# Walter0807/MotionBERT

Hardware: AMD Instinct MI355X
Metric: clips/sec [B,243,17,3] DSTformer fwd+bwd (higher is better)
Workload: dtype bf16; 1 GPU; MotionBERT full DSTformer (dim_feat 512, depth 5, 8 heads, mlp_ratio 2) train step: fwd + bwd + AdamW, 64 clips/GPU x T=243 x J=17, random-init weights, pose loss (mpjpe + 0.5 n_mpjpe + 20 velocity, fused kernel), one-launch flat AdamW; global_batch=64, frames=243, parallelism=dp1

## Files before the change

### motionbert_amd/csrc/attention.hip

```cpp
#include "attention_common.h"

template <bool SHARED> struct AttnBlock { static constexpr int THREADS = SHARED ? 512 : 256, WAVES = THREADS / 64; };
constexpr int MBX_ATTN_KV_THREADS = 256;
template <bool SHARED> struct AttnBlockKV { static constexpr int THREADS = SHARED ? MBX_ATTN_KV_THREADS : 256, WAVES = THREADS / 64; };


template <typename T, int HD, bool SHARED, bool DROP = false>
__global__ __launch_bounds__(AttnBlock<SHARED>::THREADS, (sizeof(T) == 2 && !DROP) ? 4 : 1) void attn_fwd_kernel(const T* __restrict__ qkv, T* __restrict__ o, float* __restrict__ lse,
                                                       int Tn, int J, int H, float scale, int mode, int nprob, int KP, MbxDrop dr) {
    constexpr bool IS_BF = sizeof(T) == 2;
    constexpr int KSTR = rm_stride<T>(HD);
    extern __shared__ __attribute__((aligned(16))) char smem[];
    const int tid = threadIdx.x, lane = tid & 63, wave = tid >> 6, g = lane >> 5;
    const int C = H * HD, C3 = 3 * C;
    constexpr int VSTR = KSTR;
    const int KBYTES = KP * KSTR;
    const int VBYTES = KP * VSTR;
    int prob = SHARED ? (int)blockIdx.x : (int)blockIdx.x * 4 + wave;
    const bool pvalid = prob < nprob;
    prob = min(prob, nprob - 1);
    const Prob P = decode_prob(prob, mode, Tn, J, H);
    const int gtid = SHARED ? tid : lane, gsize = SHARED ? AttnBlock<SHARED>::THREADS : 64;
    char* kt = smem + (SHARED ? 0 : wave * (KBYTES + VBYTES));
    char* vt = kt + KBYTES;
// ... 398 lines not shown
                a1 = wave_halves<WaveAdd>(a1); a2 = wave_halves<WaveAdd>(a2);
                b1 = wave_halves<WaveAdd>(b1); b2 = wave_halves<WaveAdd>(b2);
                if (rvalid && g == 0) {
                    const size_t Mtot = (size_t)(nprob / H) * P.L;
                    *reinterpret_cast<float2*>(st_part + ((size_t)(2 * P.h) * Mtot + tok) * 2) = make_float2(a1, a2);
                    *reinterpret_cast<float2*>(st_part + ((size_t)(2 * P.h + 1) * Mtot + tok) * 2) = make_float2(b1, b2);
                }
            }
        }
        if (!stats) {
            store_rowfrag<T, HD>(reinterpret_cast<T*>(vt + (size_t)i * RSTR), dk, 1.0f, g);
            store_rowfrag<T, HD>(reinterpret_cast<T*>(qt + (size_t)i * RSTR), dv, 1.0f, g);
        }
    }
    if (pvalid) {
        constexpr int CH = HD * (int)sizeof(T) / 16;
        T* ob = dqkv + P.tok0 * C3 + (size_t)P.h * HD;
        const char* sa = stats ? qt : kt;
        const char* sb = stats ? kt : vt;
        const char* sc = stats ? vt : qt;
        for (int idx = lane; idx < P.L * CH; idx += 64) {
            const int r = idx / CH, ch = idx % CH, off = r * RSTR + ch * 16;
            const uint4 a = *reinterpret_cast<const uint4*>(sa + off);
            const uint4 b = *reinterpret_cast<const uint4*>(sb + off);
            const uint4 c = *reinterpret_cast<const uint4*>(sc + off);
            if (sizeof(T) == 4 && dq_lo) {
                const size_t eo = P.tok0 * C3 + (size_t)P.h * HD + (size_t)r * rstride + ch * 4;
                bf16_t* const hi = reinterpret_cast<bf16_t*>(dqkv);
                const float va[4] = {__uint_as_float(a.x), __uint_as_float(a.y), __uint_as_float(a.z), __uint_as_float(a.w)};
                const float vb[4] = {__uint_as_float(b.x), __uint_as_float(b.y), __uint_as_float(b.z), __uint_as_float(b.w)};
                const float vc[4] = {__uint_as_float(c.x), __uint_as_float(c.y), __uint_as_float(c.z), __uint_as_float(c.w)};
                store4_planes(hi + eo, dq_lo + eo, va);
                store4_planes(hi + eo + C, dq_lo + eo + C, vb);
                store4_planes(hi + eo + 2 * C, dq_lo + eo + 2 * C, vc);
                continue;
            }
            T* dst = ob + (size_t)r * rstride + ch * (16 / (int)sizeof(T));
            *reinterpret_cast<uint4*>(dst) = a;
            *reinterpret_cast<uint4*>(dst + C) = b;
            *reinterpret_cast<uint4*>(dst + 2 * C) = c;
        }
    }
}

__device__ __forceinline__ bf16_t* qt_row(char* tile, int row, int stride) { return reinterpret_cast<bf16_t*>(tile + (size_t)row * stride); }
template <int HD>
__device__ __forceinline__ void mma_rows_ldsb(const char* tile, int stride, int row0, const char* brow, int lane, f32x16_t& acc) {
    const char* p = tile + (size_t)(row0 + (lane & 31)) * stride + (lane >> 5) * 16;
#pragma unroll
    for (int s = 0; s < HD / 16; ++s) {
        const bf16x8_t a = *reinterpret_cast<const bf16x8_t*>(p + s * 32);
        const bf16x8_t b = *reinterpret_cast<const bf16x8_t*>(brow + s * 32);
        acc = __builtin_amdgcn_mfma_f32_32x32x16_bf16(a, b, acc, 0, 0, 0);
    }
}

struct Raw4b {
    static __device__ __forceinline__ void unpack(const uint2& r, float (&v)[4]) {
        v[0] = __uint_as_float(r.x << 16); v[1] = __uint_as_float(r.x & 0xffff0000u);
        v[2] = __uint_as_float(r.y << 16); v[3] = __uint_as_float(r.y & 0xffff0000u);
    }
};
#ifndef MBX_ATTN_DBG
#define MBX_ATTN_DBG 0
#endif
#ifdef MBX_ATTN_TRACE
__device__ long long* g_attn_trace;
#define AT_TS(slot_) do { if (threadIdx.x == 0) ats[slot_] = (long long)wall_clock64(); __builtin_amdgcn_sched_barrier(0); } while (0)
#else
#define AT_TS(slot_) do { } while (0)
#endif
template <int HD, bool STATS>
__global__ __launch_bounds__(1024, 1) void attn_bwd_fused_kernel(const bf16_t* __restrict__ qkv, const bf16_t* __restrict__ o,
                                                                 const bf16_t* __restrict__ d_o, const float* __restrict__ lse,
                                                                 bf16_t* __restrict__ dqkv, int Tn, int J, int H, float scale,
                                                                 int mode, int nprob, int KP, const float* __restrict__ st_bias,
                                                                 const float* __restrict__ st_rsum, float* __restrict__ st_part) {
    typedef bf16_t T;
    constexpr int RSTR = rm_stride<T>(HD), CH = HD / 8;
    extern __shared__ __attribute__((aligned(16))) char smem[];
#ifdef MBX_ATTN_TRACE
    long long ats[8] = {0, 0, 0, 0, 0, 0, 0, 0};
#endif
    AT_TS(0);
    const int tid = threadIdx.x, lane = tid & 63, wave = __builtin_amdgcn_readfirstlane(tid >> 6), g = lane >> 5;
    const int C = H * HD, C3 = 3 * C;
    const Prob P = decode_prob((int)blockIdx.x, mode, Tn, J, H);
    const int TB = KP * RSTR;
    char* qt = smem;
    char* kt = qt + TB;
    char* vt = kt + TB;
    char* dot_ = vt + TB;
    float* lse_s = reinterpret_cast<float*>(dot_ + TB);
    float* del_s = lse_s + KP;
    uint4* vec = reinterpret_cast<uint4*>(del_s + KP);
    const size_t rstride = (size_t)P.tstep * C3, ostride = (size_t)P.tstep * C;
    const T* qbase = qkv + P.tok0 * C3 + (size_t)P.h * HD;
    const T* dobase = d_o + P.tok0 * C + (size_t)P.h * HD;
    const T* obase = o + P.tok0 * C + (size_t)P.h * HD;
    if (STATS) fill_stat_vec<HD>(vec, st_rsum, st_bias, C, P.h, tid, 1024);

    for (int i0 = tid; i0 < KP * CH; i0 += 2048) {
        uint4 v[2][4], vo[2];
        float sl[2] = {0.f, 0.f};
#pragma unroll
        for (int u = 0; u < 2; ++u) {
            const int idx = i0 + u * 1024, row = idx / CH, ch = idx % CH;
#pragma unroll
            for (int t = 0; t < 4; ++t) v[u][t] = make_uint4(0u, 0u, 0u, 0u);
            vo[u] = make_uint4(0u, 0u, 0u, 0u);
            if (idx < KP * CH && row < P.L && !(MBX_ATTN_DBG & 4)) {
                const T* r3 = qbase + (size_t)row * rstride + ch * 8;
                v[u][0] = *reinterpret_cast<const uint4*>(r3);
                v[u][1] = *reinterpret_cast<const uint4*>(r3 + C);
                v[u][2] = *reinterpret_cast<const uint4*>(r3 + 2 * C);
                v[u][3] = *reinterpret_cast<const uint4*>(dobase + (size_t)row * ostride + ch * 8);
                vo[u] = *reinterpret_cast<const uint4*>(obase + (size_t)row * ostride + ch * 8);
                if (ch == 0) sl[u] = lse[(P.tok0 + (size_t)row * P.tstep) * H + P.h];
            }
        }
#pragma unroll
        for (int u = 0; u < 2; ++u) {
            const int idx = i0 + u * 1024, row = idx / CH, ch = idx % CH;
            if (idx < KP * CH) {
                const int off = row * RSTR + ch * 16;
                *reinterpret_cast<uint4*>(qt + off) = v[u][0];
                *reinterpret_cast<uint4*>(kt + off) = v[u][1];
                *reinterpret_cast<uint4*>(vt + off) = v[u][2];
                *reinterpret_cast<uint4*>(dot_ + off) = v[u][3];
            }
        }
        AT_TS(1);
#pragma unroll
        for (int u = 0; u < 2; ++u) {
            const int idx = i0 + u * 1024, row = idx / CH, ch = idx % CH;
            float x[4], y[4], dl = 0.f;
            Raw4b::unpack(make_uint2(v[u][3].x, v[u][3].y), x); Raw4b::unpack(make_uint2(vo[u].x, vo[u].y), y);
            dl = fmaf(x[0], y[0], fmaf(x[1], y[1], fmaf(x[2], y[2], fmaf(x[3], y[3], dl))));
            Raw4b::unpack(make_uint2(v[u][3].z, v[u][3].w), x); Raw4b::unpack(make_uint2(vo[u].z, vo[u].w), y);
            dl = fmaf(x[0], y[0], fmaf(x[1], y[1], fmaf(x[2], y[2], fmaf(x[3], y[3], dl))));
            dl += dpp_mov<0xB1>(dl, dl);
            dl += dpp_mov<0x4E>(dl, dl);
            if (CH == 8) dl += dpp_mov<0x141>(dl, dl);
            if (ch == 0 && idx < KP * CH) {
                lse_s[row] = sl[u] * 1.44269504088896341f;
                del_s[row] = dl;
            }
        }
    }
    __syncthreads();
    AT_TS(2);

    const int nfr = (P.L + 31) / 32;
    const float c2 = scale * 1.44269504088896341f;
    f32x16_t acc[2 * (HD / 32)];
#pragma unroll
    for (int a = 0; a < 2 * (HD / 32); ++a)
#pragma unroll
        for (int r = 0; r < 16; ++r) acc[a][r] = 0.f;
    const bool qrole = wave >= 8;
    const int blk = wave & 7, row = blk * 32 + (lane & 31);
    if (blk < nfr && !(MBX_ATTN_DBG & 1)) {
        if (qrole) {
            BReg<T, HD> qreg, doreg;
            qreg.load(reinterpret_cast<const T*>(qt + (size_t)row * RSTR), g, true);
            doreg.load(reinterpret_cast<const T*>(dot_ + (size_t)row * RSTR), g, true);
            const float delta = del_s[row], lq2 = lse_s[row];
            for (int f = 0; f < nfr; ++f) {
                f32x16_t s, dp;
#pragma unroll
                for (int r = 0; r < 16; ++r) { s[r] = 0.f; dp[r] = 0.f; }
                MmaRows<T, HD>::run(kt, RSTR, 32 * f, qreg, lane, s);
                MmaRows<T, HD>::run(vt, RSTR, 32 * f, doreg, lane, dp);
#pragma unroll
                for (int r = 0; r < 16; ++r) {
                    const float p = __builtin_amdgcn_exp2f(fmaf(s[r], c2, -lq2));
                    s[r] = p * (dp[r] - delta);
                }
#pragma unroll
                for (int df = 0; df < HD / 32; ++df) MmaCols<T>::run(kt, RSTR, df * 32, f, s, lane, acc[df]);
            }
        } else {
            int boff = row * RSTR + g * 16;
            for (int f = 0; f < nfr; ++f) {
                asm volatile("" : "+v"(boff));
                f32x16_t s, dp;
#pragma unroll
                for (int r = 0; r < 16; ++r) { s[r] = 0.f; dp[r] = 0.f; }
                mma_rows_ldsb<HD>(qt, RSTR, 32 * f, kt + boff, lane, s);
                mma_rows_ldsb<HD>(dot_, RSTR, 32 * f, vt + boff, lane, dp);
#pragma unroll
                for (int qd = 0; qd < 4; ++qd) {
                    const int q0 = 32 * f + 8 * qd + 4 * g;
                    const float4 l4 = *reinterpret_cast<const float4*>(lse_s + q0);
                    const float4 d4 = *reinterpret_cast<const float4*>(del_s + q0);
                    const float la[4] = {l4.x, l4.y, l4.z, l4.w}, da[4] = {d4.x, d4.y, d4.z, d4.w};
#pragma unroll
                    for (int e = 0; e < 4; ++e) {
                        const int r = 4 * qd + e;
                        const float p = __builtin_amdgcn_exp2f(fmaf(s[r], c2, -la[e]));
                        dp[r] = p * (dp[r] - da[e]);
                        s[r] = p;
                    }
                }
#pragma unroll
                for (int df = 0; df < HD / 32; ++df) {
                    MmaCols<T>::run(dot_, RSTR, df * 32, f, s, lane, acc[HD / 32 + df]);
                    MmaCols<T>::run(qt, RSTR, df * 32, f, dp, lane, acc[df]);
                }
            }
        }
#pragma unroll
        for (int a = 0; a < HD / 32; ++a)
#pragma unroll
            for (int r = 0; r < 16; ++r) acc[a][r] *= scale;
    }
    AT_TS(3);
#ifdef MBX_ATTN_TRACE
    if (g_attn_trace != nullptr && (threadIdx.x & 63) == 0) g_attn_trace[(size_t)gridDim.x * 9 + (size_t)blockIdx.x * 16 + (threadIdx.x >> 6)] = (long long)wall_clock64();
#endif
    __syncthreads();
    AT_TS(4);
    int tid2 = threadIdx.x;
    asm volatile("" : "+v"(tid2));
    const int g2 = (tid2 >> 5) & 1, row2 = blk * 32 + (tid2 & 31);
    const bool qrole2 = wave >= 8;
    if (blk < nfr) {
        if (STATS) {
            float p1 = 0.f, p2 = 0.f;
            if (qrole2) {
                store_rowfrag_dot<HD>(qt_row(qt, row2, RSTR), reinterpret_cast<const f32x16_t (&)[HD / 32]>(acc[0]), g2, vec, p1, p2);
            } else {
                store_rowfrag_dot<HD>(qt_row(kt, row2, RSTR), reinterpret_cast<const f32x16_t (&)[HD / 32]>(acc[0]), g2, vec + HD / 4, p1, p2);
                store_rowfrag_dot<HD>(qt_row(vt, row2, RSTR), reinterpret_cast<const f32x16_t (&)[HD / 32]>(acc[HD / 32]), g2, vec + 2 * (HD / 4), p1, p2);
            }
            p1 = wave_halves<WaveAdd>(p1);
            p2 = wave_halves<WaveAdd>(p2);
            if (g2 == 0 && row2 < P.L) {
                const size_t Mtot = (size_t)(nprob / H) * P.L;
                *reinterpret_cast<float2*>(st_part + ((size_t)(2 * P.h + (qrole2 ? 0 : 1)) * Mtot + P.tok0 + (size_t)row2 * P.tstep) * 2) = make_float2(p1, p2);
            }
        } else if (qrole2) {
            store_rowfrag<T, HD>(reinterpret_cast<T*>(qt + (size_t)row2 * RSTR), reinterpret_cast<const f32x16_t (&)[HD / 32]>(acc[0]), 1.0f, g2);
        } else {
            store_rowfrag<T, HD>(reinterpret_cast<T*>(kt + (size_t)row2 * RSTR), reinterpret_cast<const f32x16_t (&)[HD / 32]>(acc[0]), 1.0f, g2);
            store_rowfrag<T, HD>(reinterpret_cast<T*>(vt + (size_t)row2 * RSTR), reinterpret_cast<const f32x16_t (&)[HD / 32]>(acc[HD / 32]), 1.0f, g2);
        }
    }
    __syncthreads();
    AT_TS(5);
    T* obase3 = dqkv + P.tok0 * C3 + (size_t)P.h * HD;
    for (int i0 = tid2; i0 < KP * CH; i0 += 2048) {
        uint4 v[2][3];
#pragma unroll
        for (int u = 0; u < 2; ++u) {
            const int idx = min(i0 + u * 1024, KP * CH - 1), off = (idx / CH) * RSTR + (idx % CH) * 16;
            v[u][0] = *reinterpret_cast<const uint4*>(qt + off);
            v[u][1] = *reinterpret_cast<const uint4*>(kt + off);
            v[u][2] = *reinterpret_cast<const uint4*>(vt + off);
        }
#pragma unroll
        for (int u = 0; u < 2; ++u) {
            const int idx = i0 + u * 1024, r = idx / CH, ch = idx % CH;
            if (idx < KP * CH && r < P.L && !(MBX_ATTN_DBG & 2)) {
                T* r3 = obase3 + (size_t)r * rstride + ch * 8;
                *reinterpret_cast<uint4*>(r3) = v[u][0];
                *reinterpret_cast<uint4*>(r3 + C) = v[u][1];
                *reinterpret_cast<uint4*>(r3 + 2 * C) = v[u][2];
            }
        }
    }
#ifdef MBX_ATTN_TRACE
    AT_TS(6);
    asm volatile("s_waitcnt vmcnt(0)" ::: "memory");
    AT_TS(7);
    if (g_attn_trace != nullptr && threadIdx.x == 0) {
        long long* const tr = g_attn_trace + (size_t)blockIdx.x * 9;
#pragma unroll
        for (int k = 0; k < 8; ++k) tr[k] = ats[k];
        tr[8] = (long long)__builtin_amdgcn_s_getreg(63492) | ((long long)__builtin_amdgcn_s_getreg(63508) << 32);
    }
#endif
}

static int check_attn_args(const char* who, int B, int T, int J, int H, int hd, int mode, int dtype) {
    MBX_CHECK_ARG(B > 0 && T > 0 && J > 0 && H > 0, "%s: bad shape", who);
    MBX_CHECK_ARG(hd == 32 || hd == 64, "%s: head dim %d unsupported (32 or 64)", who, hd);
    MBX_CHECK_ARG(mode == MBX_ATTN_SPATIAL || mode == MBX_ATTN_TEMPORAL, "%s: unknown mode %d", who, mode);
    MBX_CHECK_ARG(dtype == MBX_BF16 || dtype == MBX_F32, "%s: unknown dtype %d", who, dtype);
    return 0;
}

static int make_drop(const char* who, float p, uint64_t seed, MbxDrop& dr) {
    MBX_CHECK_ARG(p >= 0.f && p < 1.f, "%s: dropout rate %g outside [0, 1)", who, (double)p);
    dr.seed_lo = (uint32_t)seed;
    dr.seed_hi = (uint32_t)(seed >> 32);
    dr.thresh = p > 0.f ? (uint32_t)fminf(p * 4294967296.0f, 4294967295.0f) : 0u;
    dr.scale = p > 0.f ? 1.0f / (1.0f - p) : 1.0f;
    return 0;
}

template <typename T, int HD, bool SHARED, bool DROP>
static int launch_fwd(const void* qkv, void* o, float* lse, int Tn, int J, int H, float scale, int mode, int nprob, int KP, hipStream_t s,
                      const MbxDrop& dr) {
    constexpr bool IS_BF = sizeof(T) == 2;
    const size_t per = (size_t)2 * KP * rm_stride<T>(HD);
    const size_t shm = SHARED ? per : 4 * per;
    auto kern = attn_fwd_kernel<T, HD, SHARED, DROP>;
    if (set_lds(kern, shm, "attn_fwd")) return 1;
    const int grid = SHARED ? nprob : (nprob + 3) / 4;
    hipLaunchKernelGGL(kern, dim3(grid), dim3(AttnBlock<SHARED>::THREADS), shm, s, (const T*)qkv, (T*)o, lse, Tn, J, H, scale, mode, nprob, KP, dr);
    MBX_LAUNCH_CHECK("attn_fwd");
    return 0;
}

static int attn_fwd_impl(const void* qkv, void* o, float* lse, int B, int T, int J, int H, int hd, float scale, int mode,
                         int dtype, void* stream, const MbxDrop& dr) {
    MBX_CHECK_ARG(qkv && o && lse, "attn_fwd: null pointer");
    MBX_CHECK_ARG(scale > 0.f, "attn_fwd: scale must be positive (the running max is taken over the raw scores), got %g", (double)scale);
    if (check_attn_args("attn_fwd", B, T, J, H, hd, mode, dtype)) return 1;
    const int L = mode == MBX_ATTN_SPATIAL ? J : T;
    if (L > 256) return mbx_launch_attn_fwd_stream(qkv, o, lse, B, T, J, H, hd, scale, mode, dtype, (hipStream_t)stream, dr);
    const int nprob = mode == MBX_ATTN_SPATIAL ? B * T * H : B * J * H;
    const int KP = ((L + 31) / 32) * 32;
    const bool shared = KP > 32;
    hipStream_t s = (hipStream_t)stream;
#define MBX_FWD2(TT, HDV, DR)                                                                        \
    (shared ? launch_fwd<TT, HDV, true, DR>(qkv, o, lse, T, J, H, scale, mode, nprob, KP, s, dr)       \
            : launch_fwd<TT, HDV, false, DR>(qkv, o, lse, T, J, H, scale, mode, nprob, KP, s, dr))
#define MBX_FWD(TT, HDV) (dr.thresh ? MBX_FWD2(TT, HDV, true) : MBX_FWD2(TT, HDV, false))
    if (dtype == MBX_BF16) return hd == 64 ? MBX_FWD(bf16_t, 64) : MBX_FWD(bf16_t, 32);
    return hd == 64 ? MBX_FWD(float, 64) : MBX_FWD(float, 32);
#undef MBX_FWD
#undef MBX_FWD2
}
extern "C" int mbx_attn_fwd(const void* qkv, void* o, float* lse, int B, int T, int J, int H, int hd, float scale, int mode,
                            int dtype, void* stream) {
    MbxDrop dr;
    make_drop("attn_fwd", 0.f, 0, dr);
    return attn_fwd_impl(qkv, o, lse, B, T, J, H, hd, scale, mode, dtype, stream, dr);
}
extern "C" int mbx_attn_fwd_drop(const void* qkv, void* o, float* lse, int B, int T, int J, int H, int hd, float scale, int mode,
                                 int dtype, float p, uint64_t seed, void* stream) {
    MbxDrop dr;
    if (make_drop("attn_fwd_drop", p, seed, dr)) return 1;
    return attn_fwd_impl(qkv, o, lse, B, T, J, H, hd, scale, mode, dtype, stream, dr);
}

template <typename T, int HD, bool SHARED, bool DROP>
static int launch_bwd(const void* qkv, const void* o, const void* d_o, const float* lse, void* dqkv, int Tn, int J, int H,
                      float scale, int mode, int nprob, int KP, hipStream_t s, const MbxDrop& dr, void* dq_lo) {
    constexpr bool IS_BF = sizeof(T) == 2;
    const int RSTR = rm_stride<T>(HD);
    const size_t per_dq = (size_t)2 * KP * RSTR;
    const size_t per_dkv = (size_t)2 * KP * RSTR + 2 * KP * 4;
    const int grid = SHARED ? nprob : (nprob + 3) / 4;
    auto k1 = attn_bwd_dq_kernel<T, HD, SHARED, DROP>;
    auto k2 = attn_bwd_dkv_kernel<T, HD, SHARED, DROP>;
    const size_t shm1 = SHARED ? per_dq : 4 * per_dq, shm2 = SHARED ? per_dkv : 4 * per_dkv;
    if (set_lds(k1, shm1, "attn_bwd_dq") || set_lds(k2, shm2, "attn_bwd_dkv")) return 1;
    hipLaunchKernelGGL(k1, dim3(grid), dim3(AttnBlock<SHARED>::THREADS), shm1, s, (const T*)qkv, (const T*)o, (const T*)d_o, lse, (T*)dqkv, Tn, J, H, scale, mode, nprob, KP, dr, (bf16_t*)dq_lo);
    MBX_LAUNCH_CHECK("attn_bwd_dq");
    hipLaunchKernelGGL(k2, dim3(grid), dim3(AttnBlockKV<SHARED>::THREADS), shm2, s, (const T*)qkv, (const T*)o, (const T*)d_o, lse, (T*)dqkv, Tn, J, H, scale, mode, nprob, KP, dr, (bf16_t*)dq_lo);
    MBX_LAUNCH_CHECK("attn_bwd_dkv");
    return 0;
}

#ifdef MBX_ATTN_TRACE
#define MBX_ATTN_TRACE_SET(s_) do { static long long* const tb = [] { const char* e = getenv("MBX_TRACE_BUF"); return e ? (long long*)strtoull(e, nullptr, 0) : (long long*)nullptr; }(); \
                                    (void)hipMemcpyToSymbolAsync(HIP_SYMBOL(g_attn_trace), &tb, sizeof(tb), 0, hipMemcpyHostToDevice, (s_)); } while (0)
#else
#define MBX_ATTN_TRACE_SET(s_) do { } while (0)
#endif
static int attn_bwd_impl(const void* qkv, const void* o, const void* d_o, const float* lse, void* dqkv, int B, int T, int J,
                         int H, int hd, float scale, int mode, int dtype, void* stream, const float* st_bias, const float* st_rsum,
                         float* st_part, const MbxDrop& dr, void* dq_lo = nullptr) {
    MBX_CHECK_ARG(qkv && o && d_o && lse && dqkv, "attn_bwd: null pointer");
    MBX_CHECK_ARG(!dq_lo || dtype == MBX_F32, "attn_bwd: operand planes are an output form of the fp32 kernels");
    MBX_CHECK_ARG(!(st_part && dr.thresh), "attn_bwd: the row dots of the folded LayerNorm backward and dropout do not combine");
    if (check_attn_args("attn_bwd", B, T, J, H, hd, mode, dtype)) return 1;
    const int L = mode == MBX_ATTN_SPATIAL ? J : T;
    if (L > 256)
        return mbx_launch_attn_bwd_stream(qkv, o, d_o, lse, dqkv, B, T, J, H, hd, scale, mode, dtype, (hipStream_t)stream, st_bias, st_rsum,
                                          st_part, dr, dq_lo);
    const int nprob = mode == MBX_ATTN_SPATIAL ? B * T * H : B * J * H;
    const int KP = ((L + 31) / 32) * 32;
    const bool shared = KP > 32;
    hipStream_t s = (hipStream_t)stream;
    if (shared && dtype == MBX_BF16 && !dr.thresh) {
        const size_t shm = (size_t)4 * KP * rm_stride<bf16_t>(hd) + 2 * KP * 4 + 3 * hd * 4;
        if (shm <= 160 * 1024) {
#define MBX_BWD_FUSED(HDV)                                                                                            \
    do {                                                                                                              \
        auto k = st_part ? attn_bwd_fused_kernel<HDV, true> : attn_bwd_fused_kernel<HDV, false>;                     \
        if (set_lds(k, shm, "attn_bwd_fused")) return 1;                                                              \
        MBX_ATTN_TRACE_SET(s);                                                                                        \
        hipLaunchKernelGGL(k, dim3(nprob), dim3(1024), shm, s, (const bf16_t*)qkv, (const bf16_t*)o, (const bf16_t*)d_o, lse, \
                           (bf16_t*)dqkv, T, J, H, scale, mode, nprob, KP, st_bias, st_rsum, st_part);                \
        MBX_LAUNCH_CHECK("attn_bwd_fused");                                                                           \
        return 0;                                                                                                     \
    } while (0)
            if (hd == 64) MBX_BWD_FUSED(64); else MBX_BWD_FUSED(32);
#undef MBX_BWD_FUSED
        }
    }
    if (!shared) {
#define MBX_BWD_SMALL2(TT, HDV, DR)                                                                                   \
    do {                                                                                                              \
        const size_t shm = (size_t)4 * (4 * 32 * rm_stride<TT>(HDV) + 2 * 32 * 4);                                    \
        auto k = attn_bwd_small_kernel<TT, HDV, DR>;                                                                  \
        if (set_lds(k, shm, "attn_bwd_small")) return 1;                                                              \
        hipLaunchKernelGGL(k, dim3((nprob + 3) / 4), dim3(256), shm, s, (const TT*)qkv, (const TT*)o, (const TT*)d_o, lse, \
                           (TT*)dqkv, T, J, H, scale, mode, nprob, st_bias, st_rsum, st_part, dr, (bf16_t*)dq_lo);   \
        MBX_LAUNCH_CHECK("attn_bwd_small");                                                                           \
        return 0;                                                                                                     \
    } while (0)
#define MBX_BWD_SMALL(TT, HDV) do { if (dr.thresh) MBX_BWD_SMALL2(TT, HDV, true); else MBX_BWD_SMALL2(TT, HDV, false); } while (0)
        if (dtype == MBX_BF16) { if (hd == 64) MBX_BWD_SMALL(bf16_t, 64); else MBX_BWD_SMALL(bf16_t, 32); }
        else { if (hd == 64) MBX_BWD_SMALL(float, 64); else MBX_BWD_SMALL(float, 32); }
#undef MBX_BWD_SMALL
#undef MBX_BWD_SMALL2
    }
    MBX_CHECK_ARG(!st_part, "attn_bwd_stats: this shape runs the two-kernel backward, which has no row-dot output");
#define MBX_BWD2(TT, HDV, DR)                                                                                         \
    (shared ? launch_bwd<TT, HDV, true, DR>(qkv, o, d_o, lse, dqkv, T, J, H, scale, mode, nprob, KP, s, dr, dq_lo)    \
            : launch_bwd<TT, HDV, false, DR>(qkv, o, d_o, lse, dqkv, T, J, H, scale, mode, nprob, KP, s, dr, dq_lo))
#define MBX_BWD(TT, HDV) (dr.thresh ? MBX_BWD2(TT, HDV, true) : MBX_BWD2(TT, HDV, false))
    if (dtype == MBX_BF16) return hd == 64 ? MBX_BWD(bf16_t, 64) : MBX_BWD(bf16_t, 32);
    return hd == 64 ? MBX_BWD(float, 64) : MBX_BWD(float, 32);
#undef MBX_BWD
#undef MBX_BWD2
}

extern "C" int mbx_attn_bwd(const void* qkv, const void* o, const void* d_o, const float* lse, void* dqkv, int B, int T, int J,
                            int H, int hd, float scale, int mode, int dtype, void* stream) {
    MbxDrop dr;
    make_drop("attn_bwd", 0.f, 0, dr);
    return attn_bwd_impl(qkv, o, d_o, lse, dqkv, B, T, J, H, hd, scale, mode, dtype, stream, nullptr, nullptr, nullptr, dr);
}
extern "C" int mbx_attn_bwd_planes(const void* qkv, const void* o, const void* d_o, const float* lse, void* dqkv_hi, void* dqkv_lo, int B,
                                   int T, int J, int H, int hd, float scale, int mode, float p, uint64_t seed, void* stream) {
    MBX_CHECK_ARG(dqkv_lo, "attn_bwd_planes: null pointer");
    MbxDrop dr;
    if (make_drop("attn_bwd_planes", p, seed, dr)) return 1;
    return attn_bwd_impl(qkv, o, d_o, lse, dqkv_hi, B, T, J, H, hd, scale, mode, MBX_F32, stream, nullptr, nullptr, nullptr, dr, dqkv_lo);
}
extern "C" int mbx_attn_bwd_drop(const void* qkv, const void* o, const void* d_o, const float* lse, void* dqkv, int B, int T, int J,
                                 int H, int hd, float scale, int mode, int dtype, float p, uint64_t seed, void* stream) {
    MbxDrop dr;
    if (make_drop("attn_bwd_drop", p, seed, dr)) return 1;
    return attn_bwd_impl(qkv, o, d_o, lse, dqkv, B, T, J, H, hd, scale, mode, dtype, stream, nullptr, nullptr, nullptr, dr);
}
extern "C" int mbx_attn_bwd_stats(const void* qkv, const void* o, const void* d_o, const float* lse, void* dqkv, const float* bias_f,
                                  const float* rsum, float* part, int B, int T, int J, int H, int hd, float scale, int mode,
                                  void* stream) {
    MBX_CHECK_ARG(bias_f && rsum && part, "attn_bwd_stats: null pointer");
    MBX_CHECK_ARG((reinterpret_cast<uintptr_t>(part) & 7) == 0, "attn_bwd_stats: part must be 8-byte aligned");
    MbxDrop dr;
    make_drop("attn_bwd_stats", 0.f, 0, dr);
    return attn_bwd_impl(qkv, o, d_o, lse, dqkv, B, T, J, H, hd, scale, mode, MBX_BF16, stream, bias_f, rsum, part, dr);
}
```

### motionbert_amd/csrc/attention_common.h

```cpp
#pragma once
#include "mbx_common.h"

template <typename T> struct AT;
template <> struct AT<bf16_t> { static constexpr int EPC = 8, RB = 8, SZ = 2; };
template <> struct AT<float>  { static constexpr int EPC = 4, RB = 4, SZ = 4; };

template <typename T, int HD> struct BReg;
template <int HD> struct BReg<bf16_t, HD> {
    uint4 v[HD / 16];
    __device__ __forceinline__ void load(const bf16_t* row, int g, bool valid) {
#pragma unroll
        for (int s = 0; s < HD / 16; ++s)
            v[s] = valid ? *reinterpret_cast<const uint4*>(row + 16 * s + 8 * g) : make_uint4(0u, 0u, 0u, 0u);
    }
    static __device__ __forceinline__ float dot(const BReg& a, const BReg& b) {
        float acc = 0.f;
        const uint32_t* x = reinterpret_cast<const uint32_t*>(a.v);
        const uint32_t* y = reinterpret_cast<const uint32_t*>(b.v);
#pragma unroll
        for (int i = 0; i < HD / 4; ++i) {
            acc = fmaf(__uint_as_float(x[i] << 16), __uint_as_float(y[i] << 16), acc);
            acc = fmaf(__uint_as_float(x[i] & 0xffff0000u), __uint_as_float(y[i] & 0xffff0000u), acc);
        }
        return acc;
// ... 94 lines not shown
        if (row < KP) {
            *reinterpret_cast<uint4*>(dst0 + (size_t)row * stride + ch * 16) = v0[i];
            *reinterpret_cast<uint4*>(dst1 + (size_t)row * stride + ch * 16) = v1[i];
        }
    }
}
template <typename T, int HD, int NPT = HD / AT<T>::EPC>
__device__ __forceinline__ void fill_two(char* dst0, const T* src0, size_t rs0, char* dst1, const T* src1, size_t rs1, int stride,
                                         int L, int KP, int gtid, int gsize) {
    uint4 v0[NPT], v1[NPT];
    fill_two<T, HD, NPT>(dst0, src0, rs0, dst1, src1, rs1, stride, L, KP, gtid, gsize, v0, v1);
}
template <typename T, int HD>
__device__ __forceinline__ void store_rowfrag(T* row, const f32x16_t (&acc)[HD / 32], float mul, int g) {
#pragma unroll
    for (int df = 0; df < HD / 32; ++df)
#pragma unroll
        for (int q = 0; q < 4; ++q) {
            const float v[4] = {acc[df][4 * q] * mul, acc[df][4 * q + 1] * mul, acc[df][4 * q + 2] * mul, acc[df][4 * q + 3] * mul};
            store4<T>(row + df * 32 + 8 * q + 4 * g, v);
        }
}

template <int HD>
__device__ __forceinline__ void store_rowfrag_planes(bf16_t* hi, bf16_t* lo, const f32x16_t (&acc)[HD / 32], int g) {
#pragma unroll
    for (int df = 0; df < HD / 32; ++df)
#pragma unroll
        for (int q = 0; q < 4; ++q) {
            const float v[4] = {acc[df][4 * q], acc[df][4 * q + 1], acc[df][4 * q + 2], acc[df][4 * q + 3]};
            store4_planes(hi + df * 32 + 8 * q + 4 * g, lo + df * 32 + 8 * q + 4 * g, v);
        }
}

struct Prob {
    size_t tok0;
    size_t dbase;
    int tstep, L, h;
};
__device__ __forceinline__ Prob decode_prob(int prob, int mode, int Tn, int J, int H) {
    Prob p;
    p.h = prob % H;
    const int rest = prob / H;
    if (mode == MBX_ATTN_SPATIAL) {
        p.tok0 = (size_t)rest * J; p.tstep = 1; p.L = J;
        p.dbase = ((size_t)rest * H + p.h) * J * J;
    } else {
        const int j = rest % J, b = rest / J;
        p.tok0 = (size_t)b * Tn * J + j; p.tstep = J; p.L = Tn;
        p.dbase = (((size_t)b * H + p.h) * J + j) * Tn * Tn;
    }
    return p;
}
__device__ __forceinline__ float drop_mul(const MbxDrop& dr, size_t dbase, int qi, int ki, int L) {
    const size_t idx = dbase + (size_t)qi * L + ki;
    return drop_keep(dr.seed_lo, dr.seed_hi, (uint32_t)idx, (uint32_t)(idx >> 32), dr.thresh) ? dr.scale : 0.f;
}

template <typename T> __host__ __device__ constexpr int rm_stride(int HD) { return HD * AT<T>::SZ + 16; }

template <int HD>
__device__ __forceinline__ void store_rowfrag_dot(bf16_t* __restrict__ row, const f32x16_t (&acc)[HD / 32], int g,
                                                  const uint4* __restrict__ vec, float& p1, float& p2) {
#pragma unroll
    for (int df = 0; df < HD / 32; ++df) {
        uint2 o[4];
        uint4 vv[4];
#pragma unroll
        for (int q = 0; q < 4; ++q) {
            const int d0 = df * 32 + 8 * q + 4 * g;
            o[q] = *reinterpret_cast<const uint2*>(row + d0);
            vv[q] = vec[d0 >> 2];
        }
#pragma unroll
        for (int q = 0; q < 4; ++q) {
            const int d0 = df * 32 + 8 * q + 4 * g;
            const uint32_t lo = pack_bf2(acc[df][4 * q], acc[df][4 * q + 1]), hi = pack_bf2(acc[df][4 * q + 2], acc[df][4 * q + 3]);
            p1 = dot2_bf16(lo, vv[q].x, dot2_bf16(hi, vv[q].y, p1));
            p2 = dot2_bf16(lo, o[q].x, dot2_bf16(hi, o[q].y, dot2_bf16(lo, vv[q].z, dot2_bf16(hi, vv[q].w, p2))));
            *reinterpret_cast<uint2*>(row + d0) = make_uint2(lo, hi);
        }
    }
}
template <int HD>
__device__ __forceinline__ void fill_stat_vec(uint4* vec, const float* __restrict__ rsum, const float* __restrict__ bias, int C, int h,
                                              int gtid, int gsize) {
    for (int idx = gtid; idx < 3 * HD / 4; idx += gsize) {
        const int j = idx / (HD / 4), d = (idx % (HD / 4)) * 4;
        const float4 r = *reinterpret_cast<const float4*>(rsum + j * C + h * HD + d);
        const float4 b = *reinterpret_cast<const float4*>(bias + j * C + h * HD + d);
        vec[idx] = make_uint4(pack_bf2(r.x, r.y), pack_bf2(r.z, r.w), pack_bf2(-b.x, -b.y), pack_bf2(-b.z, -b.w));
    }
}

template <typename K>
static int set_lds(K kernel, size_t bytes, const char* who) {
    if (bytes > 160 * 1024) return mbx_set_error("%s: needs %zu bytes of LDS (> 160 KiB)", who, bytes);
    return bytes > 64 * 1024 ? mbx_set_dyn_lds(reinterpret_cast<const void*>(kernel), bytes, who) : 0;
}

int mbx_launch_attn_fwd_stream(const void* qkv, void* o, float* lse, int B, int T, int J, int H, int hd, float scale, int mode, int dtype,
                               hipStream_t s, const MbxDrop& dr);
int mbx_launch_attn_bwd_stream(const void* qkv, const void* o, const void* d_o, const float* lse, void* dqkv, int B, int T, int J, int H,
                               int hd, float scale, int mode, int dtype, hipStream_t s, const float* st_bias, const float* st_rsum,
                               float* st_part, const MbxDrop& dr, void* dq_lo);
```

Baseline: 580.6 clips/s.

## Make fused attention backward persistent and prefetch next problem's tiles

The fused attention backward kernel is now launched with at most one block per CU and each block loops over several problems. While the current problem's results are written out, it issues the global loads for the next problem's Q/K/V/dO/O/LSE into registers, hiding load latency behind the store phase. Accumulators are packed to bf16 before the prefetch so fewer registers stay live, and the stats vector is refilled only when the head changes. The cost is an extra barrier per trip and more live registers. The single-pass fill also assumes KP*CH fits in two 1024-thread strides.

```diff
diff --git a/motionbert_amd/csrc/attention.hip b/motionbert_amd/csrc/attention.hip
--- a/motionbert_amd/csrc/attention.hip
+++ b/motionbert_amd/csrc/attention.hip
@@ -504,10 +504,11 @@
 #ifdef MBX_ATTN_TRACE
     long long ats[8] = {0, 0, 0, 0, 0, 0, 0, 0};
 #endif
-    AT_TS(0);
-    const int tid = threadIdx.x, lane = tid & 63, wave = __builtin_amdgcn_readfirstlane(tid >> 6), g = lane >> 5;
+    const int tid = threadIdx.x, wave = __builtin_amdgcn_readfirstlane(tid >> 6);
     const int C = H * HD, C3 = 3 * C;
-    const Prob P = decode_prob((int)blockIdx.x, mode, Tn, J, H);
+    const int grid = (int)gridDim.x, ntrip = (nprob - (int)blockIdx.x + grid - 1) / grid;
+    int prob = (int)blockIdx.x;
+    Prob P = decode_prob(prob, mode, Tn, J, H);
     const int TB = KP * RSTR;
     char* qt = smem;
     char* kt = qt + TB;
@@ -516,193 +517,235 @@
     float* lse_s = reinterpret_cast<float*>(dot_ + TB);
     float* del_s = lse_s + KP;
     uint4* vec = reinterpret_cast<uint4*>(del_s + KP);
-    const size_t rstride = (size_t)P.tstep * C3, ostride = (size_t)P.tstep * C;
-    const T* qbase = qkv + P.tok0 * C3 + (size_t)P.h * HD;
-    const T* dobase = d_o + P.tok0 * C + (size_t)P.h * HD;
-    const T* obase = o + P.tok0 * C + (size_t)P.h * HD;
-    if (STATS) fill_stat_vec<HD>(vec, st_rsum, st_bias, C, P.h, tid, 1024);
-
-    for (int i0 = tid; i0 < KP * CH; i0 += 2048) {
-        uint4 v[2][4], vo[2];
-        float sl[2] = {0.f, 0.f};
+
+    uint4 v[2][4], vo[2];
+    float sl[2];
+    auto fill_issue = [&](const Prob& Q, int t, bool any) {
+        const size_t rs = (size_t)Q.tstep * C3, os = (size_t)Q.tstep * C;
+        const T* qbase = qkv + Q.tok0 * C3 + (size_t)Q.h * HD;
+        const T* dobase = d_o + Q.tok0 * C + (size_t)Q.h * HD;
+        const T* obase = o + Q.tok0 * C + (size_t)Q.h * HD;
 #pragma unroll
         for (int u = 0; u < 2; ++u) {
-            const int idx = i0 + u * 1024, row = idx / CH, ch = idx % CH;
-#pragma unroll
-            for (int t = 0; t < 4; ++t) v[u][t] = make_uint4(0u, 0u, 0u, 0u);
+            const int idx = t + u * 1024, row = idx / CH, ch = idx % CH;
+#pragma unroll
+            for (int k = 0; k < 4; ++k) v[u][k] = make_uint4(0u, 0u, 0u, 0u);
             vo[u] = make_uint4(0u, 0u, 0u, 0u);
-            if (idx < KP * CH && row < P.L && !(MBX_ATTN_DBG & 4)) {
-                const T* r3 = qbase + (size_t)row * rstride + ch * 8;
+            sl[u] = 0.f;
+            if (any && idx < KP * CH && row < Q.L && !(MBX_ATTN_DBG & 4)) {
+                const T* r3 = qbase + (size_t)row * rs + ch * 8;
                 v[u][0] = *reinterpret_cast<const uint4*>(r3);
                 v[u][1] = *reinterpret_cast<const uint4*>(r3 + C);
                 v[u][2] = *reinterpret_cast<const uint4*>(r3 + 2 * C);
-                v[u][3] = *reinterpret_cast<const uint4*>(dobase + (size_t)row * ostride + ch * 8);
-                vo[u] = *reinterpret_cast<const uint4*>(obase + (size_t)row * ostride + ch * 8);
-                if (ch == 0) sl[u] = lse[(P.tok0 + (size_t)row * P.tstep) * H + P.h];
-            }
-        }
-#pragma unroll
-        for (int u = 0; u < 2; ++u) {
-            const int idx = i0 + u * 1024, row = idx / CH, ch = idx % CH;
-            if (idx < KP * CH) {
-                const int off = row * RSTR + ch * 16;
-                *reinterpret_cast<uint4*>(qt + off) = v[u][0];
-                *reinterpret_cast<uint4*>(kt + off) = v[u][1];
-                *reinterpret_cast<uint4*>(vt + off) = v[u][2];
-                *reinterpret_cast<uint4*>(dot_ + off) = v[u][3];
-            }
-        }
-        AT_TS(1);
-#pragma unroll
-        for (int u = 0; u < 2; ++u) {
-            const int idx = i0 + u * 1024, row = idx / CH, ch = idx % CH;
-            float x[4], y[4], dl = 0.f;
-            Raw4b::unpack(make_uint2(v[u][3].x, v[u][3].y), x); Raw4b::unpack(make_uint2(vo[u].x, vo[u].y), y);
-            dl = fmaf(x[0], y[0], fmaf(x[1], y[1], fmaf(x[2], y[2], fmaf(x[3], y[3], dl))));
-            Raw4b::unpack(make_uint2(v[u][3].z, v[u][3].w), x); Raw4b::unpack(make_uint2(vo[u].z, vo[u].w), y);
-            dl = fmaf(x[0], y[0], fmaf(x[1], y[1], fmaf(x[2], y[2], fmaf(x[3], y[3], dl))));
-            dl += dpp_mov<0xB1>(dl, dl);
-            dl += dpp_mov<0x4E>(dl, dl);
-            if (CH == 8) dl += dpp_mov<0x141>(dl, dl);
-            if (ch == 0 && idx < KP * CH) {
-                lse_s[row] = sl[u] * 1.44269504088896341f;
-                del_s[row] = dl;
-            }
-        }
-    }
-    __syncthreads();
-    AT_TS(2);
+                v[u][3] = *reinterpret_cast<const uint4*>(dobase + (size_t)row * os + ch * 8);
+                vo[u] = *reinterpret_cast<const uint4*>(obase + (size_t)row * os + ch * 8);
+                if (ch == 0) sl[u] = lse[(Q.tok0 + (size_t)row * Q.tstep) * H + Q.h];
+            }
+        }
+    };
+    fill_issue(P, tid, true);
 
     const int nfr = (P.L + 31) / 32;
     const float c2 = scale * 1.44269504088896341f;
-    f32x16_t acc[2 * (HD / 32)];
-#pragma unroll
-    for (int a = 0; a < 2 * (HD / 32); ++a)
-#pragma unroll
-        for (int r = 0; r < 16; ++r) acc[a][r] = 0.f;
     const bool qrole = wave >= 8;
-    const int blk = wave & 7, row = blk * 32 + (lane & 31);
-    if (blk < nfr && !(MBX_ATTN_DBG & 1)) {
-        if (qrole) {
-            BReg<T, HD> qreg, doreg;
-            qreg.load(reinterpret_cast<const T*>(qt + (size_t)row * RSTR), g, true);
-            doreg.load(reinterpret_cast<const T*>(dot_ + (size_t)row * RSTR), g, true);
-            const float delta = del_s[row], lq2 = lse_s[row];
-            for (int f = 0; f < nfr; ++f) {
-                f32x16_t s, dp;
-#pragma unroll
-                for (int r = 0; r < 16; ++r) { s[r] = 0.f; dp[r] = 0.f; }
-                MmaRows<T, HD>::run(kt, RSTR, 32 * f, qreg, lane, s);
-                MmaRows<T, HD>::run(vt, RSTR, 32 * f, doreg, lane, dp);
-#pragma unroll
-                for (int r = 0; r < 16; ++r) {
-                    const float p = __builtin_amdgcn_exp2f(fmaf(s[r], c2, -lq2));
-                    s[r] = p * (dp[r] - delta);
+    const int blk = wave & 7;
+
+    int vec_h = -1;
+    for (int trip = 0; trip < ntrip; ++trip) {
+#ifdef MBX_ATTN_TRACE
+#pragma unroll
+        for (int k = 0; k < 8; ++k) ats[k] = 0;
+#endif
+        AT_TS(0);
+        {
+            int t1 = threadIdx.x;
+            asm volatile("" : "+v"(t1));
+            if (STATS && P.h != vec_h) {
+                fill_stat_vec<HD>(vec, st_rsum, st_bias, C, P.h, t1, 1024);
+                vec_h = P.h;
+            }
+#pragma unroll
+            for (int u = 0; u < 2; ++u) {
+                const int idx = t1 + u * 1024, row = idx / CH, ch = idx % CH;
+                if (idx < KP * CH) {
+                    const int off = row * RSTR + ch * 16;
+                    *reinterpret_cast<uint4*>(qt + off) = v[u][0];
+                    *reinterpret_cast<uint4*>(kt + off) = v[u][1];
+                    *reinterpret_cast<uint4*>(vt + off) = v[u][2];
+                    *reinterpret_cast<uint4*>(dot_ + off) = v[u][3];
                 }
-#pragma unroll
-                for (int df = 0; df < HD / 32; ++df) MmaCols<T>::run(kt, RSTR, df * 32, f, s, lane, acc[df]);
-            }
-        } else {
-            int boff = row * RSTR + g * 16;
-            for (int f = 0; f < nfr; ++f) {
-                asm volatile("" : "+v"(boff));
-                f32x16_t s, dp;
-#pragma unroll
-                for (int r = 0; r < 16; ++r) { s[r] = 0.f; dp[r] = 0.f; }
-                mma_rows_ldsb<HD>(qt, RSTR, 32 * f, kt + boff, lane, s);
-                mma_rows_ldsb<HD>(dot_, RSTR, 32 * f, vt + boff, lane, dp);
-#pragma unroll
-                for (int qd = 0; qd < 4; ++qd) {
-                    const int q0 = 32 * f + 8 * qd + 4 * g;
-                    const float4 l4 = *reinterpret_cast<const float4*>(lse_s + q0);
-                    const float4 d4 = *reinterpret_cast<const float4*>(del_s + q0);
-                    const float la[4] = {l4.x, l4.y, l4.z, l4.w}, da[4] = {d4.x, d4.y, d4.z, d4.w};
-#pragma unroll
-                    for (int e = 0; e < 4; ++e) {
-                        const int r = 4 * qd + e;
-                        const float p = __builtin_amdgcn_exp2f(fmaf(s[r], c2, -la[e]));
-                        dp[r] = p * (dp[r] - da[e]);
-                        s[r] = p;
+            }
+            AT_TS(1);
+#pragma unroll
+            for (int u = 0; u < 2; ++u) {
+                const int idx = t1 + u * 1024, row = idx / CH, ch = idx % CH;
+                float x[4], y[4], dl = 0.f;
+                Raw4b::unpack(make_uint2(v[u][3].x, v[u][3].y), x); Raw4b::unpack(make_uint2(vo[u].x, vo[u].y), y);
+                dl = fmaf(x[0], y[0], fmaf(x[1], y[1], fmaf(x[2], y[2], fmaf(x[3], y[3], dl))));
+                Raw4b::unpack(make_uint2(v[u][3].z, v[u][3].w), x); Raw4b::unpack(make_uint2(vo[u].z, vo[u].w), y);
+                dl = fmaf(x[0], y[0], fmaf(x[1], y[1], fmaf(x[2], y[2], fmaf(x[3], y[3], dl))));
+                dl += dpp_mov<0xB1>(dl, dl);
+                dl += dpp_mov<0x4E>(dl, dl);
+                if (CH == 8) dl += dpp_mov<0x141>(dl, dl);
+                if (ch == 0 && idx < KP * CH) {
+                    lse_s[row] = sl[u] * 1.44269504088896341f;
+                    del_s[row] = dl;
+                }
+            }
+        }
+        __syncthreads();
+        AT_TS(2);
+
+        uint2 pk[2 * (HD / 32)][4];
+#pragma unroll
+        for (int a = 0; a < 2 * (HD / 32); ++a)
+#pragma unroll
+            for (int q = 0; q < 4; ++q) pk[a][q] = make_uint2(0u, 0u);
+        f32x16_t acc[2 * (HD / 32)];
+#pragma unroll
+        for (int a = 0; a < 2 * (HD / 32); ++a)
+#pragma unroll
+            for (int r = 0; r < 16; ++r) acc[a][r] = 0.f;
+        if (blk < nfr && !(MBX_ATTN_DBG & 1)) {
+            int l1 = threadIdx.x;
+            asm volatile("" : "+v"(l1));
+            l1 &= 63;
+            const int g1 = l1 >> 5, row = blk * 32 + (l1 & 31);
+            if (qrole) {
+                BReg<T, HD> qreg, doreg;
+                qreg.load(reinterpret_cast<const T*>(qt + (size_t)row * RSTR), g1, true);
+                doreg.load(reinterpret_cast<const T*>(dot_ + (size_t)row * RSTR), g1, true);
+                const float delta = del_s[row], lq2 = lse_s[row];
+                for (int f = 0; f < nfr; ++f) {
+                    f32x16_t s, dp;
+#pragma unroll
+                    for (int r = 0; r < 16; ++r) { s[r] = 0.f; dp[r] = 0.f; }
+                    MmaRows<T, HD>::run(kt, RSTR, 32 * f, qreg, l1, s);
+                    MmaRows<T, HD>::run(vt, RSTR, 32 * f, doreg, l1, dp);
+#pragma unroll
+                    for (int r = 0; r < 16; ++r) {
+                        const float p = __builtin_amdgcn_exp2f(fmaf(s[r], c2, -lq2));
+                        s[r] = p * (dp[r] - delta);
+                    }
+#pragma unroll
+                    for (int df = 0; df < HD / 32; ++df) MmaCols<T>::run(kt, RSTR, df * 32, f, s, l1, acc[df]);
+                }
+            } else {
+                int boff = row * RSTR + g1 * 16;
+                for (int f = 0; f < nfr; ++f) {
+                    asm volatile("" : "+v"(boff));
+                    f32x16_t s, dp;
+#pragma unroll
+                    for (int r = 0; r < 16; ++r) { s[r] = 0.f; dp[r] = 0.f; }
+                    mma_rows_ldsb<HD>(qt, RSTR, 32 * f, kt + boff, l1, s);
+                    mma_rows_ldsb<HD>(dot_, RSTR, 32 * f, vt + boff, l1, dp);
+#pragma unroll
+                    for (int qd = 0; qd < 4; ++qd) {
+                        const int q0 = 32 * f + 8 * qd + 4 * g1;
+                        const float4 l4 = *reinterpret_cast<const float4*>(lse_s + q0);
+                        const float4 d4 = *reinterpret_cast<const float4*>(del_s + q0);
+                        const float la[4] = {l4.x, l4.y, l4.z, l4.w}, da[4] = {d4.x, d4.y, d4.z, d4.w};
+#pragma unroll
+                        for (int e = 0; e < 4; ++e) {
+                            const int r = 4 * qd + e;
+                            const float p = __builtin_amdgcn_exp2f(fmaf(s[r], c2, -la[e]));
+                            dp[r] = p * (dp[r] - da[e]);
+                            s[r] = p;
+                        }
+                    }
+#pragma unroll
+                    for (int df = 0; df < HD / 32; ++df) {
+                        MmaCols<T>::run(dot_, RSTR, df * 32, f, s, l1, acc[HD / 32 + df]);
+                        MmaCols<T>::run(qt, RSTR, df * 32, f, dp, l1, acc[df]);
                     }
                 }
-#pragma unroll
-                for (int df = 0; df < HD / 32; ++df) {
-                    MmaCols<T>::run(dot_, RSTR, df * 32, f, s, lane, acc[HD / 32 + df]);
-                    MmaCols<T>::run(qt, RSTR, df * 32, f, dp, lane, acc[df]);
+            }
+#pragma unroll
+            for (int a = 0; a < HD / 32; ++a)
+#pragma unroll
+                for (int r = 0; r < 16; ++r) acc[a][r] *= scale;
+#pragma unroll
+            for (int a = 0; a < 2 * (HD / 32); ++a)
+#pragma unroll
+                for (int q = 0; q < 4; ++q)
+                    pk[a][q] = make_uint2(pack_bf2(acc[a][4 * q], acc[a][4 * q + 1]), pack_bf2(acc[a][4 * q + 2], acc[a][4 * q + 3]));
+        }
+        AT_TS(3);
+#ifdef MBX_ATTN_TRACE
+        if (g_attn_trace != nullptr && (threadIdx.x & 63) == 0) g_attn_trace[(size_t)nprob * 9 + (size_t)prob * 16 + (threadIdx.x >> 6)] = (long long)wall_clock64();
+#endif
+        const bool more = trip + 1 < ntrip;
+        const Prob Pn = decode_prob(more ? prob + grid : prob, mode, Tn, J, H);
+        {
+            int t3 = threadIdx.x;
+            asm volatile("" : "+v"(t3));
+            fill_issue(Pn, t3, more);
+        }
+        __syncthreads();
+        AT_TS(4);
+        int tid2 = threadIdx.x;
+        asm volatile("" : "+v"(tid2));
+        const int g2 = (tid2 >> 5) & 1, row2 = blk * 32 + (tid2 & 31);
+        const size_t rstride = (size_t)P.tstep * C3;
+        if (blk < nfr) {
+            if (STATS) {
+                float p1 = 0.f, p2 = 0.f;
+                if (qrole) {
+                    store_packed_dot<HD>(qt_row(qt, row2, RSTR), pk, 0, g2, vec, p1, p2);
+                } else {
+                    store_packed_dot<HD>(qt_row(kt, row2, RSTR), pk, 0, g2, vec + HD / 4, p1, p2);
+                    store_packed_dot<HD>(qt_row(vt, row2, RSTR), pk, HD / 32, g2, vec + 2 * (HD / 4), p1, p2);
                 }
-            }
-        }
-#pragma unroll
-        for (int a = 0; a < HD / 32; ++a)
-#pragma unroll
-            for (int r = 0; r < 16; ++r) acc[a][r] *= scale;
-    }
-    AT_TS(3);
+                p1 = wave_halves<WaveAdd>(p1);
+                p2 = wave_halves<WaveAdd>(p2);
+                if (g2 == 0 && row2 < P.L) {
+                    const size_t Mtot = (size_t)(nprob / H) * P.L;
+                    *reinterpret_cast<float2*>(st_part + ((size_t)(2 * P.h + (qrole ? 0 : 1)) * Mtot + P.tok0 + (size_t)row2 * P.tstep) * 2) = make_float2(p1, p2);
+                }
+            } else if (qrole) {
+                store_packed<HD>(qt_row(qt, row2, RSTR), pk, 0, g2);
+            } else {
+                store_packed<HD>(qt_row(kt, row2, RSTR), pk, 0, g2);
+                store_packed<HD>(qt_row(vt, row2, RSTR), pk, HD / 32, g2);
+            }
+        }
+        __syncthreads();
+        AT_TS(5);
+        T* obase3 = dqkv + P.tok0 * C3 + (size_t)P.h * HD;
+        {
+            uint4 w[2][3];
+#pragma unroll
+            for (int u = 0; u < 2; ++u) {
+                const int idx = min(tid2 + u * 1024, KP * CH - 1), off = (idx / CH) * RSTR + (idx % CH) * 16;
+                w[u][0] = *reinterpret_cast<const uint4*>(qt + off);
+                w[u][1] = *reinterpret_cast<const uint4*>(kt + off);
+                w[u][2] = *reinterpret_cast<const uint4*>(vt + off);
+            }
+#pragma unroll
+            for (int u = 0; u < 2; ++u) {
+                const int idx = tid2 + u * 1024, r = idx / CH, ch = idx % CH;
+                if (idx < KP * CH && r < P.L && !(MBX_ATTN_DBG & 2)) {
+                    T* r3 = obase3 + (size_t)r * rstride + ch * 8;
+                    *reinterpret_cast<uint4*>(r3) = w[u][0];
+                    *reinterpret_cast<uint4*>(r3 + C) = w[u][1];
+                    *reinterpret_cast<uint4*>(r3 + 2 * C) = w[u][2];
+                }
+            }
+        }
+        AT_TS(6);
 #ifdef MBX_ATTN_TRACE
-    if (g_attn_trace != nullptr && (threadIdx.x & 63) == 0) g_attn_trace[(size_t)gridDim.x * 9 + (size_t)blockIdx.x * 16 + (threadIdx.x >> 6)] = (long long)wall_clock64();
+        if (g_attn_trace != nullptr && threadIdx.x == 0) {
+            long long* const tr = g_attn_trace + (size_t)prob * 9;
+#pragma unroll
+            for (int k = 0; k < 7; ++k) tr[k] = ats[k];
+            tr[7] = (long long)blockIdx.x;
+            tr[8] = (long long)__builtin_amdgcn_s_getreg(63492) | ((long long)__builtin_amdgcn_s_getreg(63508) << 32);
+        }
 #endif
-    __syncthreads();
-    AT_TS(4);
-    int tid2 = threadIdx.x;
-    asm volatile("" : "+v"(tid2));
-    const int g2 = (tid2 >> 5) & 1, row2 = blk * 32 + (tid2 & 31);
-    const bool qrole2 = wave >= 8;
-    if (blk < nfr) {
-        if (STATS) {
-            float p1 = 0.f, p2 = 0.f;
-            if (qrole2) {
-                store_rowfrag_dot<HD>(qt_row(qt, row2, RSTR), reinterpret_cast<const f32x16_t (&)[HD / 32]>(acc[0]), g2, vec, p1, p2);
-            } else {
-                store_rowfrag_dot<HD>(qt_row(kt, row2, RSTR), reinterpret_cast<const f32x16_t (&)[HD / 32]>(acc[0]), g2, vec + HD / 4, p1, p2);
-                store_rowfrag_dot<HD>(qt_row(vt, row2, RSTR), reinterpret_cast<const f32x16_t (&)[HD / 32]>(acc[HD / 32]), g2, vec + 2 * (HD / 4), p1, p2);
-            }
-            p1 = wave_halves<WaveAdd>(p1);
-            p2 = wave_halves<WaveAdd>(p2);
-            if (g2 == 0 && row2 < P.L) {
-                const size_t Mtot = (size_t)(nprob / H) * P.L;
-                *reinterpret_cast<float2*>(st_part + ((size_t)(2 * P.h + (qrole2 ? 0 : 1)) * Mtot + P.tok0 + (size_t)row2 * P.tstep) * 2) = make_float2(p1, p2);
-            }
-        } else if (qrole2) {
-            store_rowfrag<T, HD>(reinterpret_cast<T*>(qt + (size_t)row2 * RSTR), reinterpret_cast<const f32x16_t (&)[HD / 32]>(acc[0]), 1.0f, g2);
-        } else {
-            store_rowfrag<T, HD>(reinterpret_cast<T*>(kt + (size_t)row2 * RSTR), reinterpret_cast<const f32x16_t (&)[HD / 32]>(acc[0]), 1.0f, g2);
-            store_rowfrag<T, HD>(reinterpret_cast<T*>(vt + (size_t)row2 * RSTR), reinterpret_cast<const f32x16_t (&)[HD / 32]>(acc[HD / 32]), 1.0f, g2);
-        }
-    }
-    __syncthreads();
-    AT_TS(5);
-    T* obase3 = dqkv + P.tok0 * C3 + (size_t)P.h * HD;
-    for (int i0 = tid2; i0 < KP * CH; i0 += 2048) {
-        uint4 v[2][3];
-#pragma unroll
-        for (int u = 0; u < 2; ++u) {
-            const int idx = min(i0 + u * 1024, KP * CH - 1), off = (idx / CH) * RSTR + (idx % CH) * 16;
-            v[u][0] = *reinterpret_cast<const uint4*>(qt + off);
-            v[u][1] = *reinterpret_cast<const uint4*>(kt + off);
-            v[u][2] = *reinterpret_cast<const uint4*>(vt + off);
-        }
-#pragma unroll
-        for (int u = 0; u < 2; ++u) {
-            const int idx = i0 + u * 1024, r = idx / CH, ch = idx % CH;
-            if (idx < KP * CH && r < P.L && !(MBX_ATTN_DBG & 2)) {
-                T* r3 = obase3 + (size_t)r * rstride + ch * 8;
-                *reinterpret_cast<uint4*>(r3) = v[u][0];
-                *reinterpret_cast<uint4*>(r3 + C) = v[u][1];
-                *reinterpret_cast<uint4*>(r3 + 2 * C) = v[u][2];
-            }
-        }
-    }
-#ifdef MBX_ATTN_TRACE
-    AT_TS(6);
-    asm volatile("s_waitcnt vmcnt(0)" ::: "memory");
-    AT_TS(7);
-    if (g_attn_trace != nullptr && threadIdx.x == 0) {
-        long long* const tr = g_attn_trace + (size_t)blockIdx.x * 9;
-#pragma unroll
-        for (int k = 0; k < 8; ++k) tr[k] = ats[k];
-        tr[8] = (long long)__builtin_amdgcn_s_getreg(63492) | ((long long)__builtin_amdgcn_s_getreg(63508) << 32);
-    }
-#endif
+        if (more) __syncthreads();
+        P = Pn;
+        prob += grid;
+    }
 }
 
 static int check_attn_args(const char* who, int B, int T, int J, int H, int hd, int mode, int dtype) {
@@ -812,12 +855,13 @@
     if (shared && dtype == MBX_BF16 && !dr.thresh) {
         const size_t shm = (size_t)4 * KP * rm_stride<bf16_t>(hd) + 2 * KP * 4 + 3 * hd * 4;
         if (shm <= 160 * 1024) {
+            const int cus = mbx_cu_count(), grid = nprob < cus ? nprob : cus;
 #define MBX_BWD_FUSED(HDV)                                                                                            \
     do {                                                                                                              \
         auto k = st_part ? attn_bwd_fused_kernel<HDV, true> : attn_bwd_fused_kernel<HDV, false>;                     \
         if (set_lds(k, shm, "attn_bwd_fused")) return 1;                                                              \
         MBX_ATTN_TRACE_SET(s);                                                                                        \
-        hipLaunchKernelGGL(k, dim3(nprob), dim3(1024), shm, s, (const bf16_t*)qkv, (const bf16_t*)o, (const bf16_t*)d_o, lse, \
+        hipLaunchKernelGGL(k, dim3(grid), dim3(1024), shm, s, (const bf16_t*)qkv, (const bf16_t*)o, (const bf16_t*)d_o, lse, \
                            (bf16_t*)dqkv, T, J, H, scale, mode, nprob, KP, st_bias, st_rsum, st_part);                \
         MBX_LAUNCH_CHECK("attn_bwd_fused");                                                                           \
         return 0;                                                                                                     \
diff --git a/motionbert_amd/csrc/attention_common.h b/motionbert_amd/csrc/attention_common.h
--- a/motionbert_amd/csrc/attention_common.h
+++ b/motionbert_amd/csrc/attention_common.h
@@ -200,6 +200,36 @@
         }
     }
 }
+template <int HD, int NA>
+__device__ __forceinline__ void store_packed(bf16_t* row, const uint2 (&pk)[NA][4], int a0, int g) {
+#pragma unroll
+    for (int df = 0; df < HD / 32; ++df)
+#pragma unroll
+        for (int q = 0; q < 4; ++q) *reinterpret_cast<uint2*>(row + df * 32 + 8 * q + 4 * g) = pk[a0 + df][q];
+}
+template <int HD, int NA>
+__device__ __forceinline__ void store_packed_dot(bf16_t* __restrict__ row, const uint2 (&pk)[NA][4], int a0, int g,
+                                                 const uint4* __restrict__ vec, float& p1, float& p2) {
+#pragma unroll
+    for (int df = 0; df < HD / 32; ++df) {
+        uint2 o[4];
+        uint4 vv[4];
+#pragma unroll
+        for (int q = 0; q < 4; ++q) {
+            const int d0 = df * 32 + 8 * q + 4 * g;
+            o[q] = *reinterpret_cast<const uint2*>(row + d0);
+            vv[q] = vec[d0 >> 2];
+        }
+#pragma unroll
+        for (int q = 0; q < 4; ++q) {
+            const int d0 = df * 32 + 8 * q + 4 * g;
+            const uint32_t lo = pk[a0 + df][q].x, hi = pk[a0 + df][q].y;
+            p1 = dot2_bf16(lo, vv[q].x, dot2_bf16(hi, vv[q].y, p1));
+            p2 = dot2_bf16(lo, o[q].x, dot2_bf16(hi, o[q].y, dot2_bf16(lo, vv[q].z, dot2_bf16(hi, vv[q].w, p2))));
+            *reinterpret_cast<uint2*>(row + d0) = make_uint2(lo, hi);
+        }
+    }
+}
 template <int HD>
 __device__ __forceinline__ void fill_stat_vec(uint4* vec, const float* __restrict__ rsum, const float* __restrict__ bias, int C, int h,
                                               int gtid, int gsize) {
```

New measurement: 582.9 clips/s, median of 5. About the same (+0.4%).
